# hawkn/emqx

Hardware: AMD Instinct MI355X
Metric: topic matches/sec at 10M filters (higher is better)
Workload: dtype u8/u32; 1 GPU; c3: 10M mixed-wildcard filters incl. $share groups and '$SYS' exclusion; filters=10000002, topics_per_gpu_step=1000000, global_batch=1000000, parallelism=topic-sharded x1 (trie replicated), streams=3, distinct_batches=4, table_copies=1, outputs=pairs

## Files before the change

### emqx_amd/build.py

```python
from __future__ import annotations

import os
import subprocess
from pathlib import Path

PKG = Path(__file__).resolve().parent
ROOT = PKG.parent
CSRC = PKG / "csrc"

LIB_TMATCH = PKG / "libtmatch.so"
LIB_WORK = PKG / "libtmwork.so"
LIB_BENCH = PKG / "libtmbench.so"
LIB_ORACLE = ROOT / "oracle" / "liboracle.so"

ARCH = os.environ.get("TM_OFFLOAD_ARCH", "gfx950")


KERNEL_SOURCES = ("tm_kernels.hip", "tm_host.cpp", "tm_layout.h", "tm_dev.h", "tm_scan.h")
FANOUT_SOURCE = "tm_fanout.hip"
AGGRE_SOURCE = "tm_aggre.hip"
DISPATCH_SOURCE = "tm_dispatch.hip"
SHARE_SOURCE = "tm_share.hip"
GROUP_SOURCE = "tm_group.hip"
RETAIN_SOURCE = "tm_retain.hip"
RETAIN_HOST_SOURCE = "tm_retain_host.cpp"


def source_hash() -> str:
    import hashlib
    h = hashlib.sha256()
    for name in KERNEL_SOURCES:
        h.update(name.encode())
        h.update((CSRC / name).read_bytes())
    return h.hexdigest()[:16]


def _stale(out: Path, deps) -> bool:
    if not out.exists():
        return True
    t = out.stat().st_mtime
    return any(Path(d).stat().st_mtime > t for d in deps)


def _run(cmd, cwd=None):
    r = subprocess.run(cmd, cwd=cwd, capture_output=True, text=True)
    if r.returncode != 0:
        raise RuntimeError(f"build failed: {' '.join(map(str, cmd))}\n{r.stdout}\n{r.stderr}")


def build_tmatch(force: bool = False) -> Path:
    srcs = [CSRC / "tm_host.cpp", CSRC / "tm_kernels.hip", CSRC / FANOUT_SOURCE, CSRC / AGGRE_SOURCE,
            CSRC / DISPATCH_SOURCE, CSRC / SHARE_SOURCE, CSRC / GROUP_SOURCE, CSRC / RETAIN_SOURCE,
            CSRC / RETAIN_HOST_SOURCE]
    deps = srcs + [CSRC / "tm_layout.h", CSRC / "tm_dev.h", CSRC / "tm_scan.h", CSRC / "tm_subs.h", CSRC / "tm_retain.h",
                   ROOT / "include" / "tmatch.h"]
    if force or _stale(LIB_TMATCH, deps):
        tmp = LIB_TMATCH.with_suffix(".so.tmp")
        _run(["hipcc", "-O3", "-std=c++17", f"--offload-arch={ARCH}", "-fPIC", "-shared",
              "-Wall", "-Wno-unused-function", "-o", str(tmp)] + [str(s) for s in srcs])
        os.replace(tmp, LIB_TMATCH)
    return LIB_TMATCH


def build_variant(name: str, kernel_src: str | None = None, force: bool = False,
                  host_src: str | None = None) -> Path:
    out = PKG / "variants" / f"libtmatch_{name}.so"
    out.parent.mkdir(exist_ok=True)
    kern = Path(kernel_src) if kernel_src else CSRC / "tm_kernels.hip"
    srcs = [Path(host_src) if host_src else CSRC / "tm_host.cpp", kern, CSRC / FANOUT_SOURCE, CSRC / AGGRE_SOURCE,
            CSRC / DISPATCH_SOURCE, CSRC / SHARE_SOURCE, CSRC / GROUP_SOURCE, CSRC / RETAIN_SOURCE,
            CSRC / RETAIN_HOST_SOURCE]
    deps = srcs + [CSRC / "tm_layout.h", CSRC / "tm_dev.h", CSRC / "tm_scan.h", CSRC / "tm_subs.h", CSRC / "tm_retain.h",
                   ROOT / "include" / "tmatch.h"]
    if force or _stale(out, deps):
        _run(["hipcc", "-O3", "-std=c++17", f"--offload-arch={ARCH}", "-fPIC", "-shared", "-Wall",
              "-Wno-unused-function", f"-I{CSRC}", "-o", str(out)] + [str(s) for s in srcs])
    return out


def build_work(force: bool = False) -> Path:
    src = CSRC / "workload.cpp"
    if force or _stale(LIB_WORK, [src]):
        tmp = LIB_WORK.with_suffix(".so.tmp")
        _run(["g++", "-O2", "-std=c++17", "-fPIC", "-shared", "-pthread", "-o", str(tmp), str(src)])
        os.replace(tmp, LIB_WORK)
    return LIB_WORK


def build_bench(force: bool = False) -> Path:
    src = CSRC / "hostbench.cpp"
    if force or _stale(LIB_BENCH, [src, ROOT / "include" / "tmatch.h"]):
        tmp = LIB_BENCH.with_suffix(".so.tmp")
        _run(["hipcc", "-O2", "-std=c++17", "-fPIC", "-shared", "-pthread", "-o", str(tmp), str(src), "-ldl"])
        os.replace(tmp, LIB_BENCH)
    return LIB_BENCH


def build_oracle(force: bool = False) -> Path:
    src = ROOT / "oracle" / "tm_oracle.c"
    if force or _stale(LIB_ORACLE, [src]):
        _run(["make", "-B" if force else "-s", "liboracle.so"], cwd=ROOT / "oracle")
    return LIB_ORACLE


def build_all(force: bool = False) -> None:
    build_tmatch(force)
    build_work(force)
    build_bench(force)
    build_oracle(force)


if __name__ == "__main__":
    build_all(force=True)
    print("built", LIB_TMATCH, LIB_WORK, LIB_ORACLE)
```

### emqx_amd/csrc/tm_kernels.hip

```cpp
#include "tm_dev.h"
#include "tm_scan.h"

#if defined(__HIP_DEVICE_COMPILE__) && !defined(__gfx950__)
#error "tm_kernels.hip: the tail tickets' ordering is argued for gfx950 only (see above)"
#endif

namespace tmx {


__device__ __forceinline__ uint4 ld4(const void *p) { return *reinterpret_cast<const uint4 *>(p); }
__device__ __forceinline__ uint4 ld4_once(const void *p) {
    typedef unsigned int u32x4 __attribute__((ext_vector_type(4)));
    const u32x4 v = __builtin_nontemporal_load(reinterpret_cast<const u32x4 *>(p));
    return make_uint4(v.x, v.y, v.z, v.w);
}

__device__ __forceinline__ uint32_t bloom_bit(const uint4 &n2, const uint4 &n3, uint32_t b) {
    const uint32_t j = b >> 5;
    const uint32_t w = j == 0 ? n2.z : j == 1 ? n2.w : j == 2 ? n3.x : j == 3 ? n3.y : j == 4 ? n3.z : n3.w;
    return (w >> (b & 31)) & 1u;
}

__device__ __forceinline__ uint32_t child_maybe(const DevIndex &ix, const uint4 &n1, const uint4 &n2, const uint4 &n3,
                                                uint32_t w, uint32_t h) {
    if ((n1.y & NLIT_MASK) >= WIDE_LIT)
        return n2.z == NONE ? 1u : w < ix.wcap ? (ix.wbits[n2.z + (w >> 5)] >> (w & 31)) & 1u : 0u;
    return bloom_bit(n2, n3, child_bit(h));
}


__device__ __forceinline__ void pin(uint32_t &v) { asm volatile("" : "+v"(v)); }
__device__ __forceinline__ void pin(uint2 &v) { pin(v.x); pin(v.y); }
__device__ __forceinline__ void pin(uint4 &v) { pin(v.x); pin(v.y); pin(v.z); pin(v.w); }

struct WordAcc {
    uint32_t len, b0, b1;
    uint64_t start;
    __device__ __forceinline__ void reset(uint64_t s) {
        len = 0; b0 = b1 = 0; start = s;
    }
    __device__ __forceinline__ void push(uint32_t c) {
        uint32_t v = c << ((len & 3) * 8);
        if (len < 4) b0 |= v; else if (len < 8) b1 |= v;
        len++;
    }
};

struct GlobalSrc {
    const uint8_t *g;
    __device__ __forceinline__ uint4 ld16(uint64_t p) const { return ld4_once(g + p); }
    __device__ __forceinline__ uint32_t byte(uint64_t p) const { return g[p]; }
};
struct StagedSrc {
    const uint8_t *g;
    const uint4 *lds;
    uint64_t b0;
    bool staged;
    __device__ __forceinline__ uint4 ld16(uint64_t p) const {
        return staged ? lds[(uint32_t)(p - b0) >> 4] : ld4_once(g + p);
    }
    __device__ __forceinline__ uint32_t byte(uint64_t p) const {
        return staged ? reinterpret_cast<const uint8_t *>(lds)[(uint32_t)(p - b0)] : g[p];
    }
};

template <class Src>
__device__ bool bytes_eq(const uint8_t *a, const Src &src, uint64_t b, uint32_t n) {
    for (uint32_t i = 0; i < n; i++) if (a[i] != src.byte(b + i)) return false;
    return true;
}

template <class Src>
__device__ __forceinline__ uint64_t word_hash_dev(const WordAcc &w, const Src &src) {
    if (w.len <= VINL) return word_hash_short(w.b0, w.b1, w.len);
    uint64_t h = FNV_OFF;
    for (uint32_t i = 0; i < w.len; i++) h = (h ^ src.byte(w.start + i)) * FNV_PRIME;
    return word_hash_finish(h, w.len);
}

template <class Src>
__device__ uint32_t vocab_probe(const DevIndex &ix, uint32_t slot, uint32_t tag, uint32_t len, uint32_t b0,
                                uint32_t b1, const Src &src, uint64_t start) {
    for (;;) {
        const uint4 e = ld4(ix.vocab + slot);
        if (e.y == NONE) return NONE;
        if (len <= VINL) {
            if (vocab_short_eq(e.x, e.z, e.w, len, b0, b1)) return e.y;
        } else if (e.x == tag && e.w == len && bytes_eq(ix.wpool + e.z, src, start, len)) {
            return e.y;
        }
        slot = (slot + 1) & ix.vmask;
    }
}

__device__ uint32_t vocab_probe_short(const DevIndex &ix, uint32_t slot, uint32_t len, uint32_t b0, uint32_t b1,
                                      uint32_t &tag) {
    for (;;) {
        const uint4 e = ld4(ix.vocab + slot);
        if (e.y == NONE) return NONE;
        if (vocab_short_eq(e.x, e.z, e.w, len, b0, b1)) { tag = e.x; return e.y; }
        slot = (slot + 1) & ix.vmask;
    }
}

template <class Src>
__device__ uint32_t vocab_find(const DevIndex &ix, const WordAcc &w, const Src &src) {
    const uint64_t h = word_hash_dev(w, src);
    return vocab_probe(ix, (uint32_t)h & ix.vmask, vocab_tag(h, w.len), w.len, w.b0, w.b1, src, w.start);
}

// ... 209 lines not shown
                const bool hit = vocab_short_eq(e[k].x, e[k].z, e[k].w, len, b0, b1);
                uint32_t wid = e[k].y == NONE ? NONE : hit ? e[k].y : NONE - 1;
                uint32_t tag = e[k].x;
                pin(wid);
                if (use[k]) {
                    if (wid == NONE - 1) {
                        const uint64_t h = word_hash_short(b0, b1, len);
                        wid = vocab_probe_short(ix, ((uint32_t)h + 1) & ix.vmask, len, b0, b1, tag);
                    }
                    st.set_wid(l, wid);
                    if constexpr (S::hints) park |= hints_of_level(ix, l, tag);
                }
            }
        }
        if constexpr (S::hints) st.park_hints(park);
    }
    if constexpr (S::deferred && S::need) {
      const uint32_t Lw = L >> 24;
      L &= 0xFFFFFFu;
      if (Lw < L) {
        st.set_wid(Lw, NONE);
        st.set_wid(Lw + 1, NONE);
        all_found = false;
        return RC_OK;
      }
    }
    for (uint32_t l = 0; l < L; l++) {
        const uint32_t wid = st.get_wid(l);
        all_found &= wid != NONE;
        xh = seq_hash_step(xh, wid);
    }
    xh = seq_hash_finish(xh, L);
    return RC_OK;
}

__device__ __forceinline__ int tail_list(const DevIndex &ix, uint32_t nl) {
    return nl <= MAX_LEVELS && need_levels(ix, nl) <= MID_L ? L_MID : L_DEEP;
}

template <class S>
__device__ void exact_find(const DevIndex &ix, uint64_t xh, uint32_t L, const S &st, uint32_t slot, uint32_t f,
                           uint32_t &off, uint32_t &cnt) {
    cnt = 0; off = 0;
    const uint32_t fp = exact_fp(xh);
    for (;;) {
        if (f == 0) return;
        if (f == fp) {
            const uint4 *e = reinterpret_cast<const uint4 *>(ix.exact + slot);
            uint4 a = e[0], b = e[1], c = e[2], d = e[3];
            pin(a); pin(b); pin(c); pin(d);
            if (a.x == (uint32_t)xh && a.y == (uint32_t)(xh >> 32) && a.z == L) {
                bool eq = true;
                if (L <= XINL) {
                    const uint32_t iw[XINL] = {b.z, b.w, c.x, c.y, c.z, c.w, d.x, d.y, d.z, d.w};
#pragma unroll
                    for (uint32_t l = 0; l < XINL; l++)
                        if (l < L) eq &= iw[l] == st.get_wid(l);
                } else {
                    for (uint32_t l = 0; l < L && eq; l++) eq = ix.wseq[b.y + l] == st.get_wid(l);
                }
                if (eq) { off = a.w; cnt = b.x; return; }
            }
        }
        slot = (slot + 1) & ix.xmask;
        f = ix.xfp[slot];
    }
}


enum { DFS_DONE = 0, DFS_STOP = 1, DFS_REROUTE = 2 };
template <class S, class EM>
__device__ int dfs(const DevIndex &ix, uint32_t L, bool dollar, S &st, EM &em) {
    uint32_t cur = ROOT, l = 0;
    for (;;) {
        const uint4 *np = reinterpret_cast<const uint4 *>(ix.nodes + cur);
        const uint4 n0 = np[0];
        const uint4 n1 = np[1];
        const uint4 n2 = np[2];
        const uint4 n3 = np[3];
        const bool droot = dollar && l == 0;
        const uint32_t w = l < L ? st.get_wid(l) : NONE;
        uint32_t inl = n2.x == w ? n3.x : n2.y == w ? n3.y : n2.z == w ? n3.z : n2.w == w ? n3.w : NONE;
        pin(inl);
        if (l == L) {
            if (!em(n0.w, n1.x)) return DFS_STOP;
            if (!droot && !em(n0.y, n0.z)) return DFS_STOP;
            if (n1.y & NLIT_HDESC) {
                if constexpr (!S::cuts) return DFS_REROUTE;
                st.cut(L);
            }
        } else {
            uint32_t lit = NONE;
            if (w != NONE) {
                if ((n1.y & NLIT_MASK) <= KINL) {
                    lit = inl;
                } else {
                    const uint32_t h = child_hash(w);
                    bool probe = true;
                    if constexpr (S::hints) {
                        if (n1.y & (NLIT_ANX0 | NLIT_ANX1)) {
                            const uint32_t hk = st.parked_hints() >> ((n1.y & NLIT_ANX1) ? 16 : 0);
                            if (hk & HINT_KNOWN)
                                probe = (hk & HINT_CHILD) &&
                                        hint_alive(hk & HINT_MASK, l + 1, L, l + 1 < L ? st.get_wid(l + 1) : NONE);
                        }
                    }
                    if (probe && (child_maybe(ix, n1, n2, n3, w, h) & 1u)) {
                        uint32_t slo, shi;
                        lit = ctab_find(ix, n2.x, n2.y, w, h, slo, shi);
                        if (lit != NONE && !child_alive(slo, shi, l + 1, L, l + 1 < L ? st.get_wid(l + 1) : NONE,
                                                        l + 2 < L ? st.get_wid(l + 2) : NONE))
                            lit = NONE;
                    }
                }
            }
            if (!droot && !em(n0.y, n0.z)) return DFS_STOP;
            uint32_t plus = droot || (n1.y & NLIT_HDESC) ? NONE : n0.x;
            if (plus != NONE && !child_alive(n1.z, n1.w, l + 1, L, l + 1 < L ? st.get_wid(l + 1) : NONE,
                                             l + 2 < L ? st.get_wid(l + 2) : NONE))
                plus = NONE;
            if (plus != NONE) {
                if (lit != NONE) st.push(l + 1, lit);
                st.down(l, true);
                cur = plus; l++;
                continue;
            }
            if (lit != NONE) {
                st.down(l, false);
                cur = lit; l++;
                continue;
            }
        }
        if (!st.pop(l, cur)) return DFS_DONE;
        st.popped(l);
    }
}


struct RangeEmit {
    uint2 r[RCAP];
    uint32_t cnt, nr;
    __device__ __forceinline__ bool operator()(uint32_t off, uint32_t n) {
        if (n) {
#pragma unroll
            for (uint32_t i = 0; i < RCAP; i++)
                if (nr == i) r[i] = make_uint2(off, n);
            nr++; cnt += n & RUN_CNT;
        }
        return true;
    }
    __device__ __forceinline__ void store(uint2 *rng, uint64_t n, uint64_t t) const {
#pragma unroll
        for (uint32_t i = 0; i < RCAP; i++)
            if (i < nr) __builtin_nontemporal_store((uint64_t)r[i].x | ((uint64_t)r[i].y << 32),
                                                    reinterpret_cast<uint64_t *>(rng) + (uint64_t)i * n + t);
    }
};

struct DirectEmit {
    const uint32_t *vals;
    uint32_t *out;
    uint64_t pos, cap;
    __device__ __forceinline__ bool operator()(uint32_t off, uint32_t n) {
        const uint32_t c = n & RUN_CNT;
        for (uint32_t i = 0; i < c; i++, pos++)
            if (pos < cap) out[pos] = (n & RUN_INLINE) ? off : vals[off + i];
        return true;
    }
};

struct FirstEmit {
    const uint32_t *vals;
    uint32_t v;
    bool found;
    __device__ __forceinline__ bool operator()(uint32_t off, uint32_t n) {
        if (n) { v = (n & RUN_INLINE) ? off : vals[off]; found = true; return false; }
        return true;
    }
};

template <class S, class EM, class Src>
__device__ __forceinline__ int match_topic(const DevIndex &ix, const Src &src, uint64_t beg, uint64_t end, S &st,
                                           EM &em, uint32_t *levels = nullptr) {
    uint32_t L = 0; bool dollar, allf; uint64_t xh;
    int rc = tokenize(ix, src, beg, end, st, L, dollar, xh, allf);
    if (levels) *levels = L;
    if (rc) return rc;
    st.reset();
    const uint32_t xslot = (uint32_t)xh & ix.xmask;
    const uint32_t xf = allf ? ix.xfp[xslot] : 0;
    const int d = dfs(ix, L, dollar, st, em);
    if (d == DFS_STOP) return RC_OK;
    if (d == DFS_REROUTE) {
        if (levels) *levels = L;
        return RC_DEEP;
    }
    if (allf) {
        uint32_t xoff, xcnt;
        exact_find(ix, xh, L, st, xslot, xf, xoff, xcnt);
        em(xoff, xcnt);
    }
    return RC_OK;
}

enum { MODE_COUNT = 0, MODE_FIRST = 1 };

struct Outs {
    uint8_t *err;
    uint32_t *first_val;
    uint8_t *first_found;
};

__device__ __forceinline__ void list_push_wave(const Workspace &ws, uint64_t n, int k, uint32_t t) {
    const uint32_t lane = threadIdx.x & 63;
    for (int j = 0; j < L_COUNT; j++) {
        if (!__ballot(k >= 0)) break;
        const uint64_t m = __ballot(k == j);
        if (!m) continue;
        const uint32_t leader = (uint32_t)__ffsll((unsigned long long)m) - 1;
        uint32_t base = 0;
        if (lane == leader) base = atomicAdd(&ws.list_n[j], (uint32_t)__popcll(m));
        base = (uint32_t)__shfl((int)base, (int)leader, 64);
        if (k == j) ws.lists[(uint64_t)j * n + base + (uint32_t)__popcll(m & ((1ull << lane) - 1))] = t;
    }
}

__device__ __forceinline__ void list_push(const Workspace &ws, uint64_t n, int k, uint32_t t) {
    uint32_t i = atomicAdd(&ws.list_n[k], 1u);
    ws.lists[(uint64_t)k * n + i] = t;
}

template <int MODE, class S>
__device__ int run_topic(const DevIndex &ix, const Workspace &ws, uint64_t n, const uint8_t *blob,
                         const uint64_t *offs, uint64_t t, S &st, const Outs &o, uint32_t *hits,
                         int *ovf = nullptr) {
    const uint64_t beg = offs[t], end = offs[t + 1];
    if (MODE == MODE_COUNT) {
        RangeEmit em;
        em.cnt = 0; em.nr = 0;
        uint32_t levels;
        int rc = match_topic(ix, GlobalSrc{blob}, beg, end, st, em, &levels);
        const bool toolong = rc == RC_DEEP && S::maxl == MAX_LEVELS;
        if (rc == RC_DEEP && !toolong) { *hits = levels; return rc; }
        if (rc != RC_OK) { em.cnt = 0; em.nr = 0; }
        __builtin_nontemporal_store(em.cnt, ws.cnt + t);
        __builtin_nontemporal_store(em.nr, ws.nr + t);
        em.store(ws.rng, n, t);
        __builtin_nontemporal_store((uint8_t)(rc == RC_BADARG ? 1 : (toolong ? 2 : 0)), o.err + t);
        if (em.nr > RCAP) {
            const int k = S::maxl <= MID_L ? L_OVF_MID : L_OVF_DEEP;
            if (ovf) *ovf = k; else list_push(ws, n, k, (uint32_t)t);
        }
        *hits = em.cnt;
        return rc;
    } else {
        FirstEmit em{ix.vals, 0, false};
        uint32_t levels;
        int rc = match_topic(ix, GlobalSrc{blob}, beg, end, st, em, &levels);
        const bool toolong = rc == RC_DEEP && S::maxl == MAX_LEVELS;
        if (rc == RC_DEEP && !toolong) { *hits = levels; return rc; }
        o.first_val[t] = toolong ? 0 : em.v;
        o.first_found[t] = rc == RC_BADARG ? 2 : (toolong ? 3 : (em.found ? 1 : 0));
        *hits = 0;
        return rc;
    }
}


__device__ __forceinline__ uint64_t wave_incl_scan(uint64_t v) {
    const int lane = threadIdx.x & 63;
#pragma unroll
    for (int d = 1; d < 64; d <<= 1) {
        uint64_t o = __shfl_up(v, d, 64);
        if (lane >= d) v += o;
    }
    return v;
}

enum { LBR_OK = 0, LBR_FAIL = 1 };
__device__ __forceinline__ uint64_t look_back(uint64_t *look, uint32_t vb, uint32_t tag, uint64_t sum, const LbCtl &lb,
                                              int &res) {
    const uint32_t lane = threadIdx.x & 63;
    uint64_t pre = 0;
    res = vb == lb.fail_block ? LBR_FAIL : LBR_OK;
    if (res == LBR_OK && vb > 0 && lane == 0)
        __hip_atomic_store(&look[(uint64_t)vb * LB_STRIDE], lb_word(tag, LB_AGG, sum), __ATOMIC_RELAXED,
                           __HIP_MEMORY_SCOPE_AGENT);
    uint32_t spins = 0;
    for (int64_t hi = (int64_t)vb - 1; hi >= 0 && res == LBR_OK;) {
        const int64_t j = hi - (int64_t)lane;
        uint64_t f = lb_word(tag, LB_INCL, 0);
        if (j >= 0)
            for (;;) {
                f = __hip_atomic_load(&look[(uint64_t)j * LB_STRIDE], __ATOMIC_RELAXED, __HIP_MEMORY_SCOPE_AGENT);
                if (lb_tag(f) == tag || ++spins > lb.spins) break;
                __builtin_amdgcn_s_sleep(LB_SLEEP);
            }
        if (__ballot(lb_tag(f) != tag || lb_state(f) == LB_FAIL)) { res = LBR_FAIL; break; }
        const uint64_t mi = __ballot(lb_state(f) == LB_INCL);
        const uint32_t k = mi ? (uint32_t)__ffsll((long long)mi) - 1 : 63;
        uint64_t v = lane <= k ? f & LB_VAL_MASK : 0;
        for (int d = 32; d; d >>= 1) v += __shfl_xor(v, d, 64);
        pre += v;
        if (mi) break;
        hi -= 64;
    }
    if (lane == 0)
        __hip_atomic_store(&look[(uint64_t)vb * LB_STRIDE],
                           res == LBR_OK ? lb_word(tag, LB_INCL, pre + sum) : lb_word(tag, LB_FAIL, sum),
                           __ATOMIC_RELAXED, __HIP_MEMORY_SCOPE_AGENT);
    return pre;
}

__device__ __forceinline__ uint32_t wave_excl_scan32(uint32_t v, uint32_t &total) {
    const int lane = threadIdx.x & 63;
    uint32_t inc = v;
#pragma unroll
    for (int d = 1; d < 64; d <<= 1) {
        uint32_t o = __shfl_up(inc, d, 64);
        if (lane >= d) inc += o;
    }
    total = __shfl(inc, 63, 64);
    return inc - v;
}

__device__ __forceinline__ uint64_t block_excl_scan(uint64_t v, uint64_t &total, uint64_t *s_w) {
    const int lane = threadIdx.x & 63, wv = threadIdx.x >> 6, nw = blockDim.x >> 6;
    uint64_t inc = wave_incl_scan(v);
    if (lane == 63) s_w[wv] = inc;
    __syncthreads();
// ... 160 lines not shown
        if (nn > W) { r.cant = true; break; }
        wave_sync();
        if (plus != NONE) { const uint32_t k = grp.rank(mp); sn_[k] = plus; sc_[k] = code | (1ull << sh); }
        if (lit != NONE) { const uint32_t k = np_ + grp.rank(ml); sn_[k] = lit; sc_[k] = code | (2ull << sh); }
        wave_sync();
        nst = nn;
        if (gl < nst) { node = sn_[gl]; code = sc_[gl]; }
    }

    if (!r.cant && allf && !badarg) {
        uint32_t slot = xslot, f = xf, xoff = 0, xcnt = 0;
        const uint32_t fp = exact_fp(xh);
        for (;;) {
            if (f == 0) break;
            if (f == fp) {
                const uint32_t *e = reinterpret_cast<const uint32_t *>(ix.exact + slot);
                const bool keyok = e[0] == (uint32_t)xh && e[1] == (uint32_t)(xh >> 32) && e[2] == L;
                if (keyok) {
                    const uint32_t ew = !mine ? wid : L <= XINL ? e[6 + gl] : ix.wseq[e[5] + gl];
                    if (grp.ballot(mine && ew != wid) == 0) { xoff = e[3]; xcnt = e[4]; break; }
                }
            }
            slot = (slot + 1) & ix.xmask;
            f = ix.xfp[slot];
        }
        add_hits(gl == 0 && xcnt, ~0ull, xoff, xcnt);
    }
    r.nh = nh;
    r.cant |= nh > HC;
    return r;
}

template <int MODE, int W>
__global__ __launch_bounds__(WV_BLOCK) void k_walk_wave(DevIndex ix, Workspace ws, uint64_t n,
                                                        const uint8_t *blob, const uint64_t *offs, Outs o) {
    constexpr uint32_t G = 64 / W;
    __shared__ uint32_t s_slash[WV_WAVES][64];
    __shared__ uint32_t s_node[WV_WAVES][64];
    __shared__ uint64_t s_code[WV_WAVES][64];
    __shared__ uint64_t s_hcode[WV_WAVES][64];
    __shared__ uint32_t s_hoff[WV_WAVES][64], s_hcnt[WV_WAVES][64];
    const Group<W> grp;
    const uint32_t wv = threadIdx.x >> 6, gl = grp.gl, base = grp.g * W;
    const uint64_t t = ((uint64_t)blockIdx.x * WV_WAVES + wv) * G + grp.g;
    if (t >= n) return;
    uint32_t *sl_ = s_slash[wv] + base, *sn_ = s_node[wv] + base, *hoff = s_hoff[wv] + base, *hcnt = s_hcnt[wv] + base;
    uint64_t *sc_ = s_code[wv] + base, *hcode = s_hcode[wv] + base;
    const uint64_t beg = offs[t], end = offs[t + 1];
    const GroupWalk gw = group_walk<W, W, false>(ix, grp, blob + beg, end - beg, true, sl_, sn_, sc_, hcode, hoff, hcnt);
    if (gw.cant) {
        if (gl == 0) list_push(ws, n, tail_list(ix, gw.L), (uint32_t)t);
        return;
    }
    const uint32_t nh = gw.nh; const bool badarg = gw.badarg;

    wave_sync();
    const bool hv = gl < nh;
    const uint64_t my = hv ? hcode[gl] : 0;
    uint32_t rank = 0, total = 0;
    for (uint32_t j = 0; j < nh; j++) {
        rank += hcode[j] < my;
        total += hcnt[j] & RUN_CNT;
    }
    if (MODE == MODE_COUNT) {
        if (hv && rank < RCAP) ws.rng[(uint64_t)rank * n + t] = make_uint2(hoff[gl], hcnt[gl]);
        if (gl == 0) {
            ws.cnt[t] = total;
            ws.nr[t] = nh;
            o.err[t] = badarg;
            if (total) add_tile_total(ws, t, total);
            if (nh > RCAP) list_push(ws, n, L_OVF_MID, (uint32_t)t);
        }
    } else {
        if (hv && rank == 0) o.first_val[t] = (hcnt[gl] & RUN_INLINE) ? hoff[gl] : ix.vals[hoff[gl]];
        if (gl == 0) {
            if (!nh) o.first_val[t] = 0;
            o.first_found[t] = badarg ? 2 : (nh ? 1 : 0);
        }
    }
}

struct CountEmit {
    uint64_t cnt;
    __device__ __forceinline__ bool operator()(uint32_t, uint32_t n) { cnt += n & RUN_CNT; return true; }
};

constexpr uint64_t SMALL_TOPICS = 65536;

bool one_launch_ok(const DevIndex &ix) {
    return ix.depth + 2 <= (uint32_t)MID_L && ix.xlen_max + 2 <= (uint32_t)MID_L;
}

bool small_path_ok(const DevIndex &ix, uint64_t n) { return n && n <= SMALL_TOPICS && one_launch_ok(ix); }

template <int W>
struct SmallShape {
    static constexpr uint32_t G = 64 / W;
    static constexpr uint32_t ST = WV_WAVES * G;
    static constexpr uint32_t HC = W < 16 ? 16 : W;
    static constexpr uint32_t TBQ = (W >= 16 ? SM_TB : SM_TB / 2) / 16 + 1;
};
static_assert(SmallShape<16>::ST == SM_TOPICS, "SM_TOPICS: the most blocks a small batch launches per topic");

template <int MODE, class OT, int W, bool LITE>
__global__ __launch_bounds__(WV_BLOCK) void k_walk_small(DevIndex ix, Workspace ws, uint64_t n_, const uint8_t *blob_,
                                                         const OT *offs_, Outs o, OT *hit_offs_,
                                                         uint32_t *out_, uint64_t cap_, uint32_t tag, LbCtl lb,
                                                         SmallSegs sg) {
    uint64_t n = n_, cap = cap_;
    const uint8_t *blob = blob_;
    const OT *offs = offs_;
    OT *hit_offs = hit_offs_;
    uint32_t *out = out_;
    uint32_t vb = blockIdx.x, nblk = gridDim.x, sb0 = 0;
    uint32_t k = 0;
    if (MODE == MODE_COUNT && sg.count) {
        while (k + 1 < sg.count && blockIdx.x >= sg.s[k + 1].block0) k++;
        const SmallSeg &S = sg.s[k];
        n = S.n; cap = S.cap; blob = S.blob;
        offs = static_cast<const OT *>(S.offs);
        hit_offs = static_cast<OT *>(S.hit);
        out = S.out; o.err = S.err;
        sb0 = S.block0;
        nblk = (k + 1 < sg.count ? sg.s[k + 1].block0 : gridDim.x) - sb0;
        vb = blockIdx.x - sb0;
    }
    if (MODE == MODE_COUNT && lb.ticket) {
        __shared__ uint32_t s_tk;
        if (threadIdx.x == 0) {
            const uint32_t tk = atomicAdd(&ws.list_n[SM_TICK + k], 1u);
            if (tk == nblk - 1) atomicExch(&ws.list_n[SM_TICK + k], 0u);
            s_tk = tk;
        }
        __syncthreads();
        vb = s_tk;
    }
    using SH = SmallShape<W>;
    constexpr uint32_t G = SH::G, ST = SH::ST, HC = SH::HC;
    __shared__ uint32_t s_slash[WV_WAVES][64];
    __shared__ uint32_t s_node[WV_WAVES][64];
    __shared__ uint64_t s_code[WV_WAVES][64];
    __shared__ uint64_t s_hcode[WV_WAVES][G * HC];
    __shared__ uint32_t s_hoff[WV_WAVES][G * HC], s_hcnt[WV_WAVES][G * HC];
    constexpr uint32_t FBL = LITE ? FAST_L : MID_L;
    using FbStore = LdsStore<FBL, LITE>;
    __shared__ uint32_t s_mwid[ST][FBL], s_mpend[ST][FBL + 1];
    __shared__ uint8_t s_mlen[ST][FBL];
    __shared__ uint64_t s_cnt[ST];
    __shared__ uint64_t s_base;
    __shared__ uint32_t s_fail;
    constexpr uint32_t TBQ = SH::TBQ;
    constexpr uint32_t TBQ_ALL = ST * TBQ;
    __shared__ uint4 s_tb[TBQ_ALL];
    __shared__ uint64_t s_off[ST + 1];
    __shared__ uint8_t s_err[ST], s_fbk[ST];
    __shared__ uint32_t s_vals[SM_VSTAGE];
    __shared__ uint64_t s_sum;
    if (threadIdx.x <= ST && (uint64_t)vb * ST + threadIdx.x <= n)
        s_off[threadIdx.x] = offs[(uint64_t)vb * ST + threadIdx.x];
    __syncthreads();
    const Group<W> grp;
    const uint32_t wv = threadIdx.x >> 6, gl = grp.gl, base = grp.g * W;
    const uint32_t gi = wv * G + grp.g;
    const uint64_t t = (uint64_t)vb * ST + gi;
    const bool live = t < n;
    const uint32_t hbase = grp.g * HC;
// ... 413 lines not shown
    if (ovf) nr = 0;
    uint64_t gr[RCAP];
#pragma unroll
    for (int i = 0; i < RCAP; i++)
        gr[i] = (uint32_t)i < nr ? __builtin_nontemporal_load(reinterpret_cast<const uint64_t *>(ws.rng) + (uint64_t)i * n + t) : 0;
    if (wv == 0) {
        const uint64_t b = blockIdx.x, sb = b / SUP;
        uint64_t v = 0;
        for (uint64_t i = lane; i < sb; i += 64) v += ws.sup[i];
        if (sb * SUP + lane < b) v += ws.blk[sb * SUP + lane];
        v = wave_incl_scan(v);
        if (lane == 63) s_pre = v;
    }
    uint64_t total;
    const uint64_t ex = block_excl_scan(c, total, s_w);
    const uint64_t my = s_pre + ex;
    if (blockIdx.x == gridDim.x - 1 && threadIdx.x == 0) hit_offs[n] = s_pre + total;
    if (valid) __builtin_nontemporal_store(my, hit_offs + t);
    if (lane == 63) s_end[wv] = my + c;
    __syncthreads();
    const uint64_t t0 = t - lane;
    if (t0 >= n) return;
    const uint64_t base = __shfl(my, 0, 64);
    const uint64_t endp = s_end[wv];
    const uint32_t rel = (uint32_t)(my - base);
    uint32_t R;
    const uint32_t r0 = wave_excl_scan32(ovf ? (c ? 1u : 0u) : nr, R);
    if (ovf && c) {
        s_off[wv][r0] = 0;
        s_rel[wv][r0] = rel;
        s_flg[wv][r0] = RF_SKIP;
    }
    uint32_t acc = 0;
#pragma unroll
    for (int i = 0; i < RCAP; i++) {
        if ((uint32_t)i >= nr) break;
        const uint2 g = make_uint2((uint32_t)gr[i], (uint32_t)(gr[i] >> 32));
        s_off[wv][r0 + i] = g.x;
        s_rel[wv][r0 + i] = rel + acc;
        s_flg[wv][r0 + i] = (g.y & RUN_INLINE) ? RF_INLINE : 0;
        acc += g.y & RUN_CNT;
    }
    if (lane == 0) s_rel[wv][R] = (uint32_t)(endp - base);
    __builtin_amdgcn_fence(__ATOMIC_RELEASE, "wavefront");
    __builtin_amdgcn_wave_barrier();
    __builtin_amdgcn_fence(__ATOMIC_ACQUIRE, "wavefront");
    wave_emit(ix, s_off[wv], s_rel[wv], s_flg[wv], R, base, endp, out, cap);
}

struct WalkLds {
    uint32_t wid[FAST_L * WALK_BLOCK];
    uint32_t pend[(FAST_L + 1) * WALK_BLOCK];
    uint8_t len[FAST_L * WALK_BLOCK];
};
struct SpanLds {
    uint32_t off[WR];
    uint32_t rel[WR + 1];
    uint8_t flg[WR];
};
static_assert(WALK_BLOCK == 64, "k_walk_pairs: one wave per block");

__device__ __forceinline__ uint32_t vres_k(uint64_t n) {
    const uint64_t k = (n + WALK_BLOCK - 1) / WALK_BLOCK / 128;
    return k < 1 ? 1u : (k > VRES_K ? (uint32_t)VRES_K : (uint32_t)k);
}
__device__ __forceinline__ uint64_t vres_region(uint64_t cap, uint32_t K) { return (cap - cap / 8) / K; }
__device__ __forceinline__ uint64_t vres_reserve(const Workspace &ws, uint64_t cap, uint32_t K, uint32_t g, uint32_t T) {
    const uint64_t Rg = vres_region(cap, K);
    if (g < K && Rg) {
        const uint64_t old = atomicAdd((unsigned long long *)&ws.vres[g * VRES_STRIDE], (unsigned long long)T);
        if (old + T <= Rg) return g * Rg + old;
        atomicAdd((unsigned long long *)&ws.vres[g * VRES_STRIDE + 1], (unsigned long long)T);
    }
    return K * Rg + atomicAdd((unsigned long long *)&ws.vres[VRES_POOL], (unsigned long long)T);
}

__global__ __launch_bounds__(WALK_BLOCK, 8) void k_walk_pairs(DevIndex ix, Workspace ws, uint64_t n,
                                                           const uint8_t *blob, const uint64_t *offs, uint8_t *err,
                                                           uint32_t *pairs, uint32_t *out, uint64_t cap) {
    __shared__ union { WalkLds w; SpanLds e; } s;
    const uint32_t lane = threadIdx.x;
    const uint64_t t = (uint64_t)blockIdx.x * WALK_BLOCK + lane;
    RangeEmit em;
    em.cnt = 0; em.nr = 0;
    int deep = -1, ovf = -1;
    if (t < n) {
        LdsStore<FAST_L> st{s.w.wid + lane, s.w.pend + lane, s.w.len + lane, WALK_BLOCK, 0};
        uint32_t levels;
        const int rc = match_topic(ix, GlobalSrc{blob}, offs[t], offs[t + 1], st, em, &levels);
        if (rc == RC_DEEP) {
            deep = tail_list(ix, levels);
            em.cnt = 0; em.nr = 0;
        } else {
            if (rc != RC_OK) { em.cnt = 0; em.nr = 0; }
            __builtin_nontemporal_store((uint8_t)(rc == RC_BADARG ? 1 : 0), err + t);
            if (em.nr > RCAP) ovf = L_OVF_MID;
        }
    }
    list_push_wave(ws, n, deep, (uint32_t)t);
    list_push_wave(ws, n, ovf, (uint32_t)t);
    uint32_t tot;
    const uint32_t ex = wave_excl_scan32(em.cnt, tot);
    uint64_t base = 0;
    if (lane == 0 && tot) {
        const uint32_t K = vres_k(n);
        base = vres_reserve(ws, cap, K, blockIdx.x % K, tot);
    }
    base = ((uint64_t)(uint32_t)__shfl((int)(base >> 32), 0, 64) << 32) | (uint32_t)__shfl((int)(uint32_t)base, 0, 64);
    if (t < n && deep < 0) {
        const uint64_t p = base + ex < cap ? base + ex : cap;
        const uint64_t pc = (uint64_t)(uint32_t)p | ((uint64_t)em.cnt << 32);
        __builtin_nontemporal_store(pc, reinterpret_cast<uint64_t *>(pairs) + t);
    }
    if (!tot) return;
    wave_sync();
    const bool skip = ovf >= 0;
    constexpr uint32_t VST = sizeof(s) / 4;
    if (tot <= VST) {
        uint32_t *sv = reinterpret_cast<uint32_t *>(&s);
        uint32_t p = ex;
#pragma unroll
        for (int i = 0; i < RCAP; i++) {
            if (skip || (uint32_t)i >= em.nr) break;
            const uint2 r = em.r[i];
            if (r.y & RUN_INLINE) { sv[p++] = r.x; continue; }
#pragma unroll 2
            for (uint32_t k = 0; k < (r.y & RUN_CNT); k++) sv[p++] = ix.vals[r.x + k];
        }
        wave_sync();
        for (uint32_t i = lane; i < tot; i += 64)
            if (base + i < cap) __builtin_nontemporal_store(sv[i], out + base + i);
        return;
    }
    uint32_t R;
    const uint32_t r0 = wave_excl_scan32(skip ? (em.cnt ? 1u : 0u) : em.nr, R);
    if (skip && em.cnt) {
        s.e.off[r0] = 0;
        s.e.rel[r0] = ex;
        s.e.flg[r0] = RF_SKIP;
    }
    uint32_t acc = 0;
#pragma unroll
    for (int i = 0; i < RCAP; i++) {
        if (skip || (uint32_t)i >= em.nr) break;
        s.e.off[r0 + i] = em.r[i].x;
        s.e.rel[r0 + i] = ex + acc;
        s.e.flg[r0 + i] = (em.r[i].y & RUN_INLINE) ? RF_INLINE : 0;
        acc += em.r[i].y & RUN_CNT;
    }
    if (lane == 0) s.e.rel[R] = tot;
    wave_sync();
    wave_emit(ix, s.e.off, s.e.rel, s.e.flg, R, base, base + tot, out, cap);
}

template <class S>
__device__ __forceinline__ void tail_pair(const DevIndex &ix, const Workspace &ws, uint64_t n, const uint8_t *blob,
                          const uint64_t *offs, bool live, uint64_t t, uint8_t *err, uint32_t *pairs, uint32_t *out,
                          uint64_t cap, uint32_t wave_no, S &st, SpanLds &sp) {
    uint32_t c = 0;
    if (live) {
        int ovf = -1;
        const Outs o{err, nullptr, nullptr};
        const int rc = run_topic<MODE_COUNT>(ix, ws, n, blob, offs, t, st, o, &c, &ovf);
        if (rc == RC_DEEP) c = 0;
    }
    uint32_t tot;
    const uint32_t ex = wave_excl_scan32(c, tot);
    const uint32_t lane = threadIdx.x & 63;
    uint64_t base = 0;
    if (lane == 0 && tot) {
        const uint32_t K = vres_k(n);
        base = vres_reserve(ws, cap, K, wave_no % K, tot);
    }
    base = ((uint64_t)(uint32_t)__shfl((int)(base >> 32), 0, 64) << 32) | (uint32_t)__shfl((int)(uint32_t)base, 0, 64);
    const uint64_t pos = base + ex;
    if (live)
        reinterpret_cast<uint64_t *>(pairs)[t] = (uint64_t)(uint32_t)(pos < cap ? pos : cap) | ((uint64_t)c << 32);
    if (!tot) return;
    const uint32_t nr = live && c ? ws.nr[t] : 0;
    const bool skip = nr > RCAP;
    wave_sync();
    uint32_t R;
    const uint32_t r0 = wave_excl_scan32(skip ? 1u : nr, R);
    if (skip) {
        sp.off[r0] = 0;
        sp.rel[r0] = ex;
        sp.flg[r0] = RF_SKIP;
    }
    uint32_t acc = 0;
    for (uint32_t i = 0; !skip && i < nr; i++) {
        const uint64_t g = reinterpret_cast<const uint64_t *>(ws.rng)[(uint64_t)i * n + t];
        sp.off[r0 + i] = (uint32_t)g;
        sp.rel[r0 + i] = ex + acc;
        sp.flg[r0 + i] = ((uint32_t)(g >> 32) & RUN_INLINE) ? RF_INLINE : 0;
        acc += (uint32_t)(g >> 32) & RUN_CNT;
    }
    if (lane == 0) sp.rel[R] = tot;
    wave_sync();
    wave_emit(ix, sp.off, sp.rel, sp.flg, R, base, base + tot, out, cap);
    wave_sync();
    if (skip) {
        DirectEmit de{ix.vals, out, pos, cap};
        match_topic(ix, GlobalSrc{blob}, offs[t], offs[t + 1], st, de);
    }
}

__global__ __launch_bounds__(MID_BLOCK) void k_tail_pairs(DevIndex ix, Workspace ws, uint64_t n, const uint8_t *blob,
                                                          const uint64_t *offs, uint8_t *err, uint32_t *pairs,
                                                          uint32_t *out, uint64_t cap, uint32_t mid_grid) {
    __shared__ union { MidLds w; SpanLds e; } s;
    static_assert(MID_BLOCK == 64, "one wave per tail block");
    if (blockIdx.x < mid_grid) {
        LdsStore<MID_L> st = mid_store(s.w);
        const uint32_t cnt = ws.list_n[L_MID];
        const uint32_t *lst = ws.lists + (uint64_t)L_MID * n;
        for (uint32_t i0 = blockIdx.x * MID_BLOCK; i0 < cnt; i0 += mid_grid * MID_BLOCK) {
            const uint32_t i = i0 + threadIdx.x;
            tail_pair(ix, ws, n, blob, offs, i < cnt, i < cnt ? lst[i] : 0, err, pairs, out, cap, i0 / MID_BLOCK, st,
                      s.e);
        }
        const uint32_t co = ws.list_n[L_OVF_MID];
        const uint32_t *lo = ws.lists + (uint64_t)L_OVF_MID * n;
        for (uint32_t i = blockIdx.x * MID_BLOCK + threadIdx.x; i < co; i += mid_grid * MID_BLOCK) {
            const uint64_t t = lo[i];
            DirectEmit de{ix.vals, out, pairs[2 * t], cap};
            match_topic(ix, GlobalSrc{blob}, offs[t], offs[t + 1], st, de);
        }
    } else {
        const uint32_t lane = (blockIdx.x - mid_grid) * 64 + threadIdx.x;
        GlobalStore st = deep_store(ws, lane);
        const uint32_t cnt = ws.list_n[L_DEEP];
// ... 535 lines not shown
```

Baseline: 4.701 billion topic matches/s.

## Pack match-range slots into shift registers and hoist wildcard emit in DFS

Replaces the per-topic range emitter, which used uint2 slots written through a dynamic index, with a shift-register HitSlots structure. Offsets stay in one array and 16-bit counts with an inline flag are packed two per word, so slots stay in VGPRs with fewer registers and no scratch spill from indexed writes. The '#' emit in the DFS is moved ahead of the level check, and the bloom bit test becomes a 64-bit shift with a three-way select. Counts are now capped at 15 bits, with larger runs forced into the overflow path, and emit order inside the DFS changes slightly, which could affect the ordering of output pairs.

```diff
diff --git a/emqx_amd/build.py b/emqx_amd/build.py
--- a/emqx_amd/build.py
+++ b/emqx_amd/build.py
@@ -16,7 +16,7 @@
 ARCH = os.environ.get("TM_OFFLOAD_ARCH", "gfx950")
 
 
-KERNEL_SOURCES = ("tm_kernels.hip", "tm_host.cpp", "tm_layout.h", "tm_dev.h", "tm_scan.h")
+KERNEL_SOURCES = ("tm_kernels.hip", "tm_host.cpp", "tm_layout.h", "tm_dev.h", "tm_scan.h", "tm_hits.h")
 FANOUT_SOURCE = "tm_fanout.hip"
 AGGRE_SOURCE = "tm_aggre.hip"
 DISPATCH_SOURCE = "tm_dispatch.hip"
@@ -52,8 +52,8 @@
     srcs = [CSRC / "tm_host.cpp", CSRC / "tm_kernels.hip", CSRC / FANOUT_SOURCE, CSRC / AGGRE_SOURCE,
             CSRC / DISPATCH_SOURCE, CSRC / SHARE_SOURCE, CSRC / GROUP_SOURCE, CSRC / RETAIN_SOURCE,
             CSRC / RETAIN_HOST_SOURCE]
-    deps = srcs + [CSRC / "tm_layout.h", CSRC / "tm_dev.h", CSRC / "tm_scan.h", CSRC / "tm_subs.h", CSRC / "tm_retain.h",
-                   ROOT / "include" / "tmatch.h"]
+    deps = srcs + [CSRC / "tm_layout.h", CSRC / "tm_dev.h", CSRC / "tm_scan.h", CSRC / "tm_hits.h", CSRC / "tm_subs.h",
+                   CSRC / "tm_retain.h", ROOT / "include" / "tmatch.h"]
     if force or _stale(LIB_TMATCH, deps):
         tmp = LIB_TMATCH.with_suffix(".so.tmp")
         _run(["hipcc", "-O3", "-std=c++17", f"--offload-arch={ARCH}", "-fPIC", "-shared",
@@ -70,8 +70,8 @@
     srcs = [Path(host_src) if host_src else CSRC / "tm_host.cpp", kern, CSRC / FANOUT_SOURCE, CSRC / AGGRE_SOURCE,
             CSRC / DISPATCH_SOURCE, CSRC / SHARE_SOURCE, CSRC / GROUP_SOURCE, CSRC / RETAIN_SOURCE,
             CSRC / RETAIN_HOST_SOURCE]
-    deps = srcs + [CSRC / "tm_layout.h", CSRC / "tm_dev.h", CSRC / "tm_scan.h", CSRC / "tm_subs.h", CSRC / "tm_retain.h",
-                   ROOT / "include" / "tmatch.h"]
+    deps = srcs + [CSRC / "tm_layout.h", CSRC / "tm_dev.h", CSRC / "tm_scan.h", CSRC / "tm_hits.h", CSRC / "tm_subs.h",
+                   CSRC / "tm_retain.h", ROOT / "include" / "tmatch.h"]
     if force or _stale(out, deps):
         _run(["hipcc", "-O3", "-std=c++17", f"--offload-arch={ARCH}", "-fPIC", "-shared", "-Wall",
               "-Wno-unused-function", f"-I{CSRC}", "-o", str(out)] + [str(s) for s in srcs])
diff --git a/emqx_amd/csrc/tm_hits.h b/emqx_amd/csrc/tm_hits.h
--- /dev/null
+++ b/emqx_amd/csrc/tm_hits.h
@@ -0,0 +1,74 @@
+#pragma once
+#include "tm_layout.h"
+
+#if defined(__clang__)
+#define TM_NT_STORE(v, p) __builtin_nontemporal_store((v), (p))
+#else
+#define TM_NT_STORE(v, p) (*(p) = (v))
+#endif
+
+namespace tmx {
+
+constexpr uint32_t HS_INLINE = 0x8000u;
+constexpr uint32_t HS_CNT = 0x7FFFu;
+
+template <int CAP>
+struct HitSlots {
+    static_assert(CAP >= 2 && CAP % 2 == 0, "two 16-bit fields per word");
+    uint32_t x[CAP];
+    uint32_t c[CAP / 2];
+    uint32_t cnt, nr;
+
+    TM_HD void clear() { cnt = 0; nr = 0; }
+    TM_HD void begin() {
+        for (int j = 0; j < CAP / 2; j++) {
+#ifdef __HIP_DEVICE_COMPILE__
+            asm volatile("" : "=v"(c[j]));
+#else
+            c[j] = 0;
+#endif
+        }
+    }
+
+    TM_HD bool operator()(uint32_t off, uint32_t n) {
+        if (n) {
+            const uint32_t k = n & RUN_CNT;
+#ifdef __HIP_DEVICE_COMPILE__
+#pragma unroll
+#endif
+            for (int i = CAP - 1; i > 0; i--) x[i] = x[i - 1];
+            x[0] = off;
+#ifdef __HIP_DEVICE_COMPILE__
+#pragma unroll
+#endif
+            for (int j = CAP / 2 - 1; j > 0; j--) c[j] = c[j] << 16 | c[j - 1] >> 16;
+            c[0] = c[0] << 16 | ((n >> 16) & HS_INLINE) | (k & HS_CNT);
+            nr = k > HS_CNT ? (uint32_t)CAP + 1 : nr + 1;
+            cnt += k;
+        }
+        return true;
+    }
+
+    TM_HD bool overflowed() const { return nr > (uint32_t)CAP; }
+
+    TM_HD uint32_t field(int i) const { return (c[i >> 1] >> ((i & 1) * 16)) & 0xFFFFu; }
+    TM_HD uint32_t off(int i) const { return x[i]; }
+    TM_HD bool is_inline(int i) const { return (field(i) & HS_INLINE) != 0; }
+    TM_HD uint32_t count(int i) const { return field(i) & HS_CNT; }
+    TM_HD uint32_t run(int i) const {
+        const uint32_t f = field(i);
+        return (f & HS_CNT) | (f & HS_INLINE) << 16;
+    }
+
+    TM_HD void store(uint64_t *rng, uint64_t n, uint64_t t) const {
+        if (overflowed()) return;
+#ifdef __HIP_DEVICE_COMPILE__
+#pragma unroll
+#endif
+        for (int i = CAP - 1; i >= 0; i--)
+            if ((uint32_t)i < nr)
+                TM_NT_STORE((uint64_t)x[i] | (uint64_t)run(i) << 32, rng + (uint64_t)(nr - 1 - (uint32_t)i) * n + t);
+    }
+};
+
+}
diff --git a/emqx_amd/csrc/tm_kernels.hip b/emqx_amd/csrc/tm_kernels.hip
--- a/emqx_amd/csrc/tm_kernels.hip
+++ b/emqx_amd/csrc/tm_kernels.hip
@@ -1,5 +1,6 @@
 #include "tm_dev.h"
 #include "tm_scan.h"
+#include "tm_hits.h"
 
 #if defined(__HIP_DEVICE_COMPILE__) && !defined(__gfx950__)
 #error "tm_kernels.hip: the tail tickets' ordering is argued for gfx950 only (see above)"
@@ -15,17 +16,26 @@
     return make_uint4(v.x, v.y, v.z, v.w);
 }
 
+template <bool FLAT>
 __device__ __forceinline__ uint32_t bloom_bit(const uint4 &n2, const uint4 &n3, uint32_t b) {
-    const uint32_t j = b >> 5;
-    const uint32_t w = j == 0 ? n2.z : j == 1 ? n2.w : j == 2 ? n3.x : j == 3 ? n3.y : j == 4 ? n3.z : n3.w;
-    return (w >> (b & 31)) & 1u;
-}
-
+    if constexpr (FLAT) {
+        const uint32_t q = b >> 6;
+        const uint32_t lo = q == 0 ? n2.z : q == 1 ? n3.x : n3.z;
+        const uint32_t hi = q == 0 ? n2.w : q == 1 ? n3.y : n3.w;
+        return (uint32_t)(((uint64_t)hi << 32 | lo) >> (b & 63)) & 1u;
+    } else {
+        const uint32_t j = b >> 5;
+        const uint32_t w = j == 0 ? n2.z : j == 1 ? n2.w : j == 2 ? n3.x : j == 3 ? n3.y : j == 4 ? n3.z : n3.w;
+        return (w >> (b & 31)) & 1u;
+    }
+}
+
+template <bool FLAT = false>
 __device__ __forceinline__ uint32_t child_maybe(const DevIndex &ix, const uint4 &n1, const uint4 &n2, const uint4 &n3,
                                                 uint32_t w, uint32_t h) {
     if ((n1.y & NLIT_MASK) >= WIDE_LIT)
         return n2.z == NONE ? 1u : w < ix.wcap ? (ix.wbits[n2.z + (w >> 5)] >> (w & 31)) & 1u : 0u;
-    return bloom_bit(n2, n3, child_bit(h));
+    return bloom_bit<FLAT>(n2, n3, child_bit(h));
 }
 
 
@@ -401,9 +411,9 @@
         const uint32_t w = l < L ? st.get_wid(l) : NONE;
         uint32_t inl = n2.x == w ? n3.x : n2.y == w ? n3.y : n2.z == w ? n3.z : n2.w == w ? n3.w : NONE;
         pin(inl);
+        if (l == L && !em(n0.w, n1.x)) return DFS_STOP;
+        if (!droot && !em(n0.y, n0.z)) return DFS_STOP;
         if (l == L) {
-            if (!em(n0.w, n1.x)) return DFS_STOP;
-            if (!droot && !em(n0.y, n0.z)) return DFS_STOP;
             if (n1.y & NLIT_HDESC) {
                 if constexpr (!S::cuts) return DFS_REROUTE;
                 st.cut(L);
@@ -424,7 +434,7 @@
                                         hint_alive(hk & HINT_MASK, l + 1, L, l + 1 < L ? st.get_wid(l + 1) : NONE);
                         }
                     }
-                    if (probe && (child_maybe(ix, n1, n2, n3, w, h) & 1u)) {
+                    if (probe && (child_maybe<true>(ix, n1, n2, n3, w, h) & 1u)) {
                         uint32_t slo, shi;
                         lit = ctab_find(ix, n2.x, n2.y, w, h, slo, shi);
                         if (lit != NONE && !child_alive(slo, shi, l + 1, L, l + 1 < L ? st.get_wid(l + 1) : NONE,
@@ -433,7 +443,6 @@
                     }
                 }
             }
-            if (!droot && !em(n0.y, n0.z)) return DFS_STOP;
             uint32_t plus = droot || (n1.y & NLIT_HDESC) ? NONE : n0.x;
             if (plus != NONE && !child_alive(n1.z, n1.w, l + 1, L, l + 1 < L ? st.get_wid(l + 1) : NONE,
                                              l + 2 < L ? st.get_wid(l + 2) : NONE))
@@ -456,30 +465,13 @@
 }
 
 
-struct RangeEmit {
-    uint2 r[RCAP];
-    uint32_t cnt, nr;
-    __device__ __forceinline__ bool operator()(uint32_t off, uint32_t n) {
-        if (n) {
-#pragma unroll
-            for (uint32_t i = 0; i < RCAP; i++)
-                if (nr == i) r[i] = make_uint2(off, n);
-            nr++; cnt += n & RUN_CNT;
-        }
-        return true;
-    }
-    __device__ __forceinline__ void store(uint2 *rng, uint64_t n, uint64_t t) const {
-#pragma unroll
-        for (uint32_t i = 0; i < RCAP; i++)
-            if (i < nr) __builtin_nontemporal_store((uint64_t)r[i].x | ((uint64_t)r[i].y << 32),
-                                                    reinterpret_cast<uint64_t *>(rng) + (uint64_t)i * n + t);
-    }
-};
+typedef HitSlots<RCAP> RangeEmit;
 
 struct DirectEmit {
     const uint32_t *vals;
     uint32_t *out;
     uint64_t pos, cap;
+    __device__ __forceinline__ void begin() {}
     __device__ __forceinline__ bool operator()(uint32_t off, uint32_t n) {
         const uint32_t c = n & RUN_CNT;
         for (uint32_t i = 0; i < c; i++, pos++)
@@ -492,6 +484,7 @@
     const uint32_t *vals;
     uint32_t v;
     bool found;
+    __device__ __forceinline__ void begin() {}
     __device__ __forceinline__ bool operator()(uint32_t off, uint32_t n) {
         if (n) { v = (n & RUN_INLINE) ? off : vals[off]; found = true; return false; }
         return true;
@@ -506,6 +499,7 @@
     if (levels) *levels = L;
     if (rc) return rc;
     st.reset();
+    em.begin();
     const uint32_t xslot = (uint32_t)xh & ix.xmask;
     const uint32_t xf = allf ? ix.xfp[xslot] : 0;
     const int d = dfs(ix, L, dollar, st, em);
@@ -556,7 +550,7 @@
     const uint64_t beg = offs[t], end = offs[t + 1];
     if (MODE == MODE_COUNT) {
         RangeEmit em;
-        em.cnt = 0; em.nr = 0;
+        em.clear();
         uint32_t levels;
         int rc = match_topic(ix, GlobalSrc{blob}, beg, end, st, em, &levels);
         const bool toolong = rc == RC_DEEP && S::maxl == MAX_LEVELS;
@@ -564,7 +558,7 @@
         if (rc != RC_OK) { em.cnt = 0; em.nr = 0; }
         __builtin_nontemporal_store(em.cnt, ws.cnt + t);
         __builtin_nontemporal_store(em.nr, ws.nr + t);
-        em.store(ws.rng, n, t);
+        em.store(reinterpret_cast<uint64_t *>(ws.rng), n, t);
         __builtin_nontemporal_store((uint8_t)(rc == RC_BADARG ? 1 : (toolong ? 2 : 0)), o.err + t);
         if (em.nr > RCAP) {
             const int k = S::maxl <= MID_L ? L_OVF_MID : L_OVF_DEEP;
@@ -891,6 +885,7 @@
 
 struct CountEmit {
     uint64_t cnt;
+    __device__ __forceinline__ void begin() {}
     __device__ __forceinline__ bool operator()(uint32_t, uint32_t n) { cnt += n & RUN_CNT; return true; }
 };
 
@@ -1470,7 +1465,7 @@
     const uint32_t lane = threadIdx.x;
     const uint64_t t = (uint64_t)blockIdx.x * WALK_BLOCK + lane;
     RangeEmit em;
-    em.cnt = 0; em.nr = 0;
+    em.clear();
     int deep = -1, ovf = -1;
     if (t < n) {
         LdsStore<FAST_L> st{s.w.wid + lane, s.w.pend + lane, s.w.len + lane, WALK_BLOCK, 0};
@@ -1508,12 +1503,12 @@
         uint32_t *sv = reinterpret_cast<uint32_t *>(&s);
         uint32_t p = ex;
 #pragma unroll
-        for (int i = 0; i < RCAP; i++) {
-            if (skip || (uint32_t)i >= em.nr) break;
-            const uint2 r = em.r[i];
-            if (r.y & RUN_INLINE) { sv[p++] = r.x; continue; }
+        for (int i = RCAP - 1; i >= 0; i--) {
+            if (skip || (uint32_t)i >= em.nr) continue;
+            const uint32_t ro = em.off(i), rf = em.field(i);
+            if (rf & HS_INLINE) { sv[p++] = ro; continue; }
 #pragma unroll 2
-            for (uint32_t k = 0; k < (r.y & RUN_CNT); k++) sv[p++] = ix.vals[r.x + k];
+            for (uint32_t k = 0; k < (rf & HS_CNT); k++) sv[p++] = ix.vals[ro + k];
         }
         wave_sync();
         for (uint32_t i = lane; i < tot; i += 64)
@@ -1527,14 +1522,16 @@
         s.e.rel[r0] = ex;
         s.e.flg[r0] = RF_SKIP;
     }
-    uint32_t acc = 0;
+    uint32_t acc = 0, ri = r0;
 #pragma unroll
-    for (int i = 0; i < RCAP; i++) {
-        if (skip || (uint32_t)i >= em.nr) break;
-        s.e.off[r0 + i] = em.r[i].x;
-        s.e.rel[r0 + i] = ex + acc;
-        s.e.flg[r0 + i] = (em.r[i].y & RUN_INLINE) ? RF_INLINE : 0;
-        acc += em.r[i].y & RUN_CNT;
+    for (int i = RCAP - 1; i >= 0; i--) {
+        if (skip || (uint32_t)i >= em.nr) continue;
+        const uint32_t rf = em.field(i);
+        s.e.off[ri] = em.off(i);
+        s.e.rel[ri] = ex + acc;
+        s.e.flg[ri] = (rf & HS_INLINE) ? RF_INLINE : 0;
+        acc += rf & HS_CNT;
+        ri++;
     }
     if (lane == 0) s.e.rel[R] = tot;
     wave_sync();
```

Result: no change. 4.723 billion topic matches/s (median of 5 runs) (+0.5%).
